# facebookresearch/foundpose

Hardware: AMD Instinct MI355X
Metric: detections/sec (ViT+kNN match) on 518^2 crops vs 10k-template bank (higher is better)
Workload: dtype bf16; 1 GPU; tie_order=torch

## Files before the change

### foundpose_amd/_lib.py

```python

import ctypes as C
import os

import torch

_HERE = os.path.dirname(os.path.abspath(__file__))
LIB_PATH = os.environ.get("FOUNDPOSE_AMD_LIB") or os.path.join(_HERE, "lib", "libfoundpose_amd.so")

FP_F32, FP_BF16, FP_FP8, FP_F16X3, FP_F16F8, FP_F16 = 0, 1, 2, 3, 4, 5
GEMM_SPLIT_F16F8 = 1 << 20
GEMM_F16 = 1 << 21
SPLIT_SCALE_ACT, SPLIT_SCALE_QKV, SPLIT_SCALE_HID = 16.0, 16.0, 4.0
ABI_VERSION = 20

vp, i32, i64, f32, f64, u64 = C.c_void_p, C.c_int, C.c_int64, C.c_float, C.c_double, C.c_uint64


class VitBlock(C.Structure):
    _fields_ = [(n, vp) for n in (
        "ln1_w", "ln1_b", "ln2_w", "ln2_b", "ls1", "ls2",
        "qkv_w", "proj_w", "fc1_w", "fc2_w",
        "qkv_b", "proj_b", "fc1_b", "fc2_b", "qkv_s", "proj_s", "fc1_s", "fc2_s")] + [("act_scale", f32 * 4), ("qkv_colsum", vp), ("fc1_colsum", vp)]


# ... 19 lines not shown
    "fp_normalize_rows": [vp, i64, i32, f32, vp, vp],
    "fp_knn_l2": [vp, vp, i32, vp, vp, i32, i32, i32, vp, vp, vp, vp],
    "fp_tfidf_build": [vp, vp, i32, vp, i32, vp, i32, i32, f32, i32, vp, vp, f32, vp],
    "fp_cosine_topk": [vp, vp, vp, i32, i32, vp, vp, i32, i32, i32, i32, vp, vp, vp, i32, vp],
    "fp_cosine_topk_prefiltered": [vp, vp, vp, i32, i32, vp, vp, vp, i32, i32, i32, i32, vp, vp, vp, i32, vp],
    "fp_cyclic_buddies": [vp, vp, vp, vp, i32, i32, vp, vp, vp, i32, vp, vp, vp, vp, i32, i32, i32, i32,
                          vp, vp, vp, vp, vp, vp, vp, vp, i32, vp],
    "fp_pack_records": [vp, vp, vp, vp, vp, vp, vp, vp, vp, i32, i32, i32, vp, vp],
    "fp_pnp_ransac": [vp, vp, vp, vp, i32, i32, i32, i32, f64, f64, i32, i32, u64, vp, vp, vp, vp, vp, vp, vp],
    "fp_sample_bilinear": [vp, i64, i64, i64, i64, i32, i32, i32, i32, i32, vp, vp, i32, vp, vp],
    "fp_pca_project": [vp, i32, i32, vp, i32, vp, vp, vp],
    "fp_vit_forward": [C.POINTER(VitModel), C.POINTER(VitWorkspace), vp, i32, i32, i32, i32, vp],
    "fp_vit_sample_features": [C.POINTER(VitModel), C.POINTER(VitWorkspace), i32, i32, i32, i32, i32, i32, vp, vp, i32, vp, vp],
    "fp_query_select": [vp, i32, i32, i32, vp, vp, vp, i32, vp, i32, i32, vp, vp, vp, vp, vp, vp, vp, vp, vp],
    "fp_vit_forward_prefix": [C.POINTER(VitModel), C.POINTER(VitWorkspace), vp, i32, i32, i32, i32, vp],
    "fp_vit_block_selected": [C.POINTER(VitModel), C.POINTER(VitWorkspace), i32, i32, i32, i32, vp, vp, i32, i32, vp],
    "fp_vit_sample_features_selected": [C.POINTER(VitModel), C.POINTER(VitWorkspace), i32, i32, i32, i32, i32, i32, vp, vp, i32, vp, vp, vp],
    "fp_vit_features": [C.POINTER(VitModel), C.POINTER(VitWorkspace), i32, i32, i32, vp, vp, vp],
    "fp_patchify": [vp, i32, i32, i32, i32, vp, i32, i32, vp],
    "fp_layernorm": [vp, i32, vp, vp, f32, vp, i32, i32, i32, i32, i32, i32, i32, vp],
    "fp_gemm_bf16": [vp, i32, vp, i32, i32, i32, i32, i32, vp, vp, vp, i32, i32, vp],
    "fp_gemm_bf16_ln": [vp, i32, vp, i32, i32, i32, i32, i32, vp, vp, i32, i32, vp, vp, vp, i32, vp, vp],
    "fp_gemm_resid_tile_rows": [i32, i32, i32],
    "fp_ln_finalize": [vp, i32, i32, i32, i32, f32, vp, vp],
    "fp_gemm_fp8": [vp, i32, vp, i32, i32, i32, i32, i32, vp, vp, vp, i32, i32, f32, vp],
    "fp_quantize_fp8": [vp, i32, i64, f32, vp, vp],
    "fp_gemm_split": [vp, i32, vp, i32, i32, i32, i32, i32, vp, vp, vp, i32, i32, f32, f32, vp],
    "fp_attention_split": [vp, i32, vp, i32, i32, i32, i32, i32, f32, f32, i32, vp],
    "fp_layernorm_scaled": [vp, i32, vp, vp, f32, vp, i32, i32, f32, i32, i32, vp],
    "fp_gemm_f32": [vp, i32, vp, i32, i32, i32, i32, vp, vp, vp, i32, i32, vp],
    "fp_attention": [vp, i32, vp, i32, i32, i32, i32, i32, i32, vp],
    "fp_convert_f32_to_bf16": [vp, vp, i64, vp],
    "fp_warp_crops": [vp, i32, i32, i32, i32, i32, vp, vp, i32, i32, i32, i32, vp, vp, vp],
    "fp_warp_depth": [vp, i32, i32, vp, vp, i32, i32, i32, i32, vp, vp],
    "fp_render_setup": [vp, vp, vp, i32, vp, i32, vp, i32, i32, i32, vp, vp, vp, vp, vp, vp, vp, vp, vp, vp, vp, vp],
    "fp_render_raster": [vp, vp, vp, i32, vp, i32, vp, i32, i32, i32, vp, vp, vp, vp, vp, vp, vp, vp, vp, vp, vp, vp],
    "fp_texture_mips": [vp, i32, i32, vp, vp],
    "fp_render_raster_textured": [vp, vp, vp, i32, vp, i32, vp, i32, i32, i32, vp, vp, vp, vp, vp, vp, vp, vp, vp, vp, vp, vp, vp,
                                  i32, i32, vp, vp],
    "fp_template_downsample": [vp, vp, vp, i32, i32, i32, i32, vp, vp, vp, vp, vp],
    "fp_pose_errors": [vp, i32, vp, vp, vp, vp, i32, vp, i32, vp, C.c_size_t, vp, vp, vp],
    "fp_vsd_counts": [vp, i32, vp, i32, vp, i32, i32, i32, vp, vp, i32, vp, i32, vp, C.c_size_t, vp, vp],
    "fp_featuremetric_refine": [vp, i64, i64, i64, i64, i32, i32, i32, i32, i32, vp, vp, vp, vp, vp, vp, vp, i64, vp, i32, i32, i32,
                                vp, C.c_size_t, vp, vp, vp, vp, vp, vp, vp, vp, vp],
    "fp_vis_pca_colorize": [vp, i32, i32, i32, i32, i32, i32, i32, i32, vp, vp, vp],
    "fp_vis_mask_tint": [vp, vp, i32, i32, i32, vp, vp],
# ... 130 lines not shown
```

### foundpose_amd/csrc/api.cpp

```cpp
#include <cstdarg>
#include <cstdio>
#include <cstring>
#include <cstdlib>
#include <vector>

#include "../../include/foundpose_amd.h"
#include "common.hpp"
#include "kernels.hpp"

static thread_local char g_err[512] = "";

void fp_set_error(const char* fmt, ...) {
  va_list ap;
  va_start(ap, fmt);
  vsnprintf(g_err, sizeof(g_err), fmt, ap);
  va_end(ap);
}

#define ST(s) reinterpret_cast<hipStream_t>(s)
#define TRY(expr)              \
  do {                         \
    int rc__ = (expr);         \
    if (rc__ != FP_OK) return rc__; \
  } while (0)
// ... 215 lines not shown
  return patchify_launch(images, B, H, W, patch, out, ld_out, out_dtype, ST(stream), (out_dtype == FP_DTYPE_F16X3 || out_dtype == FP_DTYPE_F16F8) ? FP_SPLIT_SCALE_ACT : 1.f);
}

int fp_layernorm(const float* x, int ld_x, const float* weight, const float* bias, float eps, void* out, int ld_out,
                 int out_dtype, int dim, int out_rows, int out_rows_per_img, int in_rows_per_img, int in_skip,
                 fp_stream_t stream) {
  FP_REQUIRE(x && weight && bias && out, "fp_layernorm: null pointer");
  LayerNormArgs a;
  memset(&a, 0, sizeof(a));
  a.x = x; a.ld_x = ld_x; a.weight = weight; a.bias = bias; a.eps = eps; a.out = out; a.ld_out = ld_out;
  a.out_dtype = out_dtype; a.out_scale = 0.f; a.dim = dim; a.out_rows = out_rows;
  a.out_rows_per_img = out_rows_per_img > 0 ? out_rows_per_img : (out_rows > 0 ? out_rows : 1);
  a.in_rows_per_img = in_rows_per_img > 0 ? in_rows_per_img : a.out_rows_per_img;
  a.in_skip = in_skip;
  return layernorm_launch(a, ST(stream));
}

int fp_gemm_bf16(const void* A, int lda, const void* W, int ldw, int M, int N, int K, int M_valid, const float* bias,
                 const float* gamma, void* out, int ldo, int epilogue, fp_stream_t stream) {
  FP_REQUIRE(A && W && out, "fp_gemm_bf16: null pointer");
  const int tile = (epilogue >> 8) & 0xfff;
  const bool f16 = (epilogue >> 21) & 1;
  epilogue &= 0xff;
  FP_REQUIRE(tile == 0 || tile == 64 || tile == 128 || tile == 256 || tile == 320, "fp_gemm_bf16: bad tile override %d", tile);

  FP_REQUIRE(epilogue == GEMM_EPI_BIAS_BF16 || epilogue == GEMM_EPI_GELU_BF16 || epilogue == GEMM_EPI_LS_RESID_F32 ||
                 epilogue == GEMM_EPI_BIAS_F32 || epilogue == GEMM_EPI_SWIGLU_BF16,
             "fp_gemm_bf16: epilogue %d is not available through this entry point", epilogue);
  FP_REQUIRE(epilogue != GEMM_EPI_LS_RESID_F32 || gamma, "fp_gemm_bf16: gamma required");
  GemmBf16Args a;
  memset(&a, 0, sizeof(a));
  a.A = reinterpret_cast<const __bf16*>(A); a.lda = lda; a.W = reinterpret_cast<const __bf16*>(W); a.ldw = ldw;
  a.M = M; a.N = N; a.K = K; a.M_valid = M_valid; a.bias = bias; a.gamma = gamma; a.out = out; a.ldo = ldo;
  a.tile_override = tile;
  return gemm_launch(f16 ? GemmFmt::F16 : GemmFmt::BF16, epilogue, a, ST(stream));
}

int fp_gemm_bf16_ln(const void* A, int lda, const void* W, int ldw, int M, int N, int K, int M_valid, const float* bias, void* out, int ldo,
                    int epilogue, const float* colsum, const float* ln_row, void* xb, int ld_xb, float* stats, fp_stream_t stream) {
  FP_REQUIRE(A && W && out && bias, "fp_gemm_bf16_ln: null pointer");
  const int tile = (epilogue >> 8) & 0xfff;
  const bool f16 = (epilogue >> 21) & 1;
  epilogue &= 0xff;
  FP_REQUIRE(tile == 0 || tile == 64 || tile == 128 || tile == 256 || tile == 320 || (tile == 352 && epilogue == GEMM_EPI_RESID_HILO), "fp_gemm_bf16_ln: bad tile override %d", tile);
  GemmBf16Args a;
  memset(&a, 0, sizeof(a));
  a.A = reinterpret_cast<const __bf16*>(A); a.lda = lda; a.W = reinterpret_cast<const __bf16*>(W); a.ldw = ldw;
  a.M = M; a.N = N; a.K = K; a.M_valid = M_valid; a.bias = bias; a.out = out; a.ldo = ldo; a.tile_override = tile;
  if (epilogue == GEMM_EPI_RESID_HILO) {
    FP_REQUIRE(xb && stats, "fp_gemm_bf16_ln: epilogue 8 needs xb, out (= the low halves) and stats");
    a.xb = reinterpret_cast<__bf16*>(xb); a.ld_xb = ld_xb; a.xl = reinterpret_cast<__bf16*>(out); a.stats_out = reinterpret_cast<float2*>(stats);
    a.out = nullptr;
  } else if (epilogue == GEMM_EPI_RESID_F32) {
    FP_REQUIRE((xb == nullptr) == (stats == nullptr), "fp_gemm_bf16_ln: xb and stats go together");
    FP_REQUIRE(!xb || (N % 128 == 0 && ld_xb >= N && ld_xb % 4 == 0), "fp_gemm_bf16_ln: N must be a multiple of 128 and ld_xb cover the row");
    a.xb = reinterpret_cast<__bf16*>(xb); a.ld_xb = ld_xb; a.stats_out = reinterpret_cast<float2*>(stats);
  } else {
    FP_REQUIRE(epilogue == GEMM_EPI_BIAS_BF16 || epilogue == GEMM_EPI_GELU_BF16 || epilogue == GEMM_EPI_SWIGLU_BF16,
               "fp_gemm_bf16_ln: epilogue %d has no folded-LayerNorm form", epilogue);
    FP_REQUIRE(colsum && ln_row, "fp_gemm_bf16_ln: colsum and ln_row are required");
    a.colsum = colsum; a.ln_stats = reinterpret_cast<const float2*>(ln_row); a.ln_eps = 1e-6f;
  }
  return gemm_launch(f16 ? GemmFmt::F16 : GemmFmt::BF16, epilogue, a, ST(stream));
}

int fp_gemm_resid_tile_rows(int M_valid, int N, int num_cus) { return gemm_resid_tile_rows(M_valid, N, num_cus); }

int fp_ln_finalize(const float* stats, int parts, int stats_stride, int rows, int dim, float eps, float* ln_row, fp_stream_t stream) {
  FP_REQUIRE(stats && ln_row && parts >= 1 && dim >= 1, "fp_ln_finalize: bad arguments");
  return ln_finalize_launch(reinterpret_cast<const float2*>(stats), parts, stats_stride, rows, dim, eps, reinterpret_cast<float2*>(ln_row), ST(stream));
}

#ifdef FP_GEMM_TIMELINE
int fp_gemm_bf16_timeline(const void* A, int lda, const void* W, int ldw, int M, int N, int K, int M_valid, const float* bias,
                          const float* gamma, void* out, int ldo, int epilogue, unsigned long long* dbg, int64_t dbg_len,
                          fp_stream_t stream) {
  FP_REQUIRE(A && W && out && dbg, "fp_gemm_bf16_timeline: null pointer");
  FP_REQUIRE(dbg_len >= 4ll * ((M + 127) / 128) * ((N + 127) / 128) * 2, "fp_gemm_bf16_timeline: stamp buffer too small");
  GemmBf16Args a;
  memset(&a, 0, sizeof(a));
  a.A = reinterpret_cast<const __bf16*>(A); a.lda = lda; a.W = reinterpret_cast<const __bf16*>(W); a.ldw = ldw;
  a.M = M; a.N = N; a.K = K; a.M_valid = M_valid; a.bias = bias; a.gamma = gamma; a.out = out; a.ldo = ldo;
  a.tile_override = (epilogue >> 8) & 0xfff;
  a.dbg = dbg;
  return gemm_launch(GemmFmt::BF16, epilogue & 0xff, a, ST(stream));
}
#endif

int fp_gemm_fp8(const void* A, int lda, const void* W, int ldw, int M, int N, int K, int M_valid, const float* bias,
// ... 635 lines not shown
```

### foundpose_amd/csrc/gemm_bf16.hip

```cpp
#include "gemm_kernel.hpp"

int gemm_resid_tile_rows(int m_valid, int n, int cus) { return resid_tile_rows(m_valid, n, cus); }

template int gemm_launch_fmt<GemmFmt::BF16>(int epi, const GemmBf16Args& a, hipStream_t st);
```

### foundpose_amd/csrc/gemm_kernel.hpp

```cpp
#pragma once
#include "common.hpp"
#include "kernels.hpp"
#include <type_traits>

namespace {

constexpr int BK = 64;

typedef __attribute__((address_space(3))) void lds_void;

FP_DEVICE int swz(int row) { return (row >> 1) & 7; }

FP_DEVICE unsigned stage_lane_offset(int ld, int lane, int parity) {
  const int row_l = lane >> 3;
  const int chunk = (lane & 7) ^ ((4 * parity + (row_l >> 1)) & 7);
  return (unsigned)(row_l * ld + chunk * 8) * 2u;
}
FP_DEVICE void stage_rows(__amdgpu_buffer_rsrc_t rsrc, unsigned voff, int ld, int row0, int k0, char* lds, int rblk) {
  const unsigned soff = (unsigned)((row0 + rblk * 8) * ld + k0) * 2u;
  __builtin_amdgcn_raw_ptr_buffer_load_lds(rsrc, (lds_void*)(lds + rblk * 1024), 16, voff, soff, 0, 0);
}

FP_DEVICE bf16x8 read_frag(const char* lds, int row, int chunk) {
  return *reinterpret_cast<const bf16x8*>(lds + row * 128 + ((chunk ^ swz(row)) << 4));
// ... 50 lines not shown
  q = __builtin_elementwise_fma(q, t, f32x2{0.15704123123125485f, 0.15704123123125485f});
  q = q * t;
  const f32x2 a = z * (z * f32x2{-1.44269504088896340736f, -1.44269504088896340736f});
  const f32x2 e = {__builtin_amdgcn_exp2f(a[0]), __builtin_amdgcn_exp2f(a[1])};
  const f32x2 erfz = __builtin_elementwise_fma(-q, e, f32x2{1.f, 1.f});
  return __builtin_elementwise_fma(hax, erfz, hx);
}

FP_DEVICE float row32_sum(float v) {
  v += __builtin_bit_cast(float, __builtin_amdgcn_update_dpp(0, __builtin_bit_cast(int, v), 0xB1, 0xF, 0xF, true));
  v += __builtin_bit_cast(float, __builtin_amdgcn_update_dpp(0, __builtin_bit_cast(int, v), 0x4E, 0xF, 0xF, true));
  v += __builtin_bit_cast(float, __builtin_amdgcn_update_dpp(0, __builtin_bit_cast(int, v), 0x124, 0xF, 0xF, true));
  v += __builtin_bit_cast(float, __builtin_amdgcn_update_dpp(0, __builtin_bit_cast(int, v), 0x128, 0xF, 0xF, true));
  v += __builtin_bit_cast(float, __builtin_amdgcn_update_dpp(0, __builtin_bit_cast(int, v), 0x142, 0xA, 0xF, true));
  return v;
}

FP_DEVICE float row16_sum(float v) {
  v += __builtin_bit_cast(float, __builtin_amdgcn_update_dpp(0, __builtin_bit_cast(int, v), 0xB1, 0xF, 0xF, true));
  v += __builtin_bit_cast(float, __builtin_amdgcn_update_dpp(0, __builtin_bit_cast(int, v), 0x4E, 0xF, 0xF, true));
  v += __builtin_bit_cast(float, __builtin_amdgcn_update_dpp(0, __builtin_bit_cast(int, v), 0x124, 0xF, 0xF, true));
  v += __builtin_bit_cast(float, __builtin_amdgcn_update_dpp(0, __builtin_bit_cast(int, v), 0x128, 0xF, 0xF, true));
  return v;
}

typedef __attribute__((ext_vector_type(8))) int i32x8;
typedef __attribute__((ext_vector_type(4))) int i32x4;

template <int EPI, int BM, int BN, int WM, int WN, GemmFmt FMT, bool F8OUT = false, int NSTAGE = 2>
__global__ __launch_bounds__(WM * WN * 64, 2) void gemm_bf16_kernel(GemmBf16Args a) {
  constexpr bool F8 = FMT == GemmFmt::FP8, SX = FMT == GemmFmt::F16F8, SP = FMT == GemmFmt::F16X3 || SX, H16 = FMT == GemmFmt::F16;
  constexpr bool SPOUT = SP && (EPI == GEMM_EPI_BIAS_BF16 || EPI == GEMM_EPI_GELU_BF16 || EPI == GEMM_EPI_SWIGLU_BF16);
  static_assert(NSTAGE == 2 || (NSTAGE == 4 && !F8 && !SP && WM * WN != 8), "the deep pipeline exists for the small bf16 / fp16 tiles");
  static_assert(!F8OUT || (F8 && (EPI == GEMM_EPI_GELU_BF16 || EPI == GEMM_EPI_SWIGLU_BF16)), "fp8 output: GELU / SwiGLU epilogues of the fp8 kernels");
  constexpr int NW = WM * WN, NT = NW * 64, MT = BM / 32, TM = (MT + WM - 1) / WM, WROWS = TM * 32, TN = BN / WN / 32;
  constexpr bool UNEVEN = MT % WM != 0;
  static_assert(BM % 32 == 0 && (!UNEVEN || (WM == 2 && FMT != GemmFmt::FP8 && FMT != GemmFmt::F16X3 && FMT != GemmFmt::F16F8)), "uneven wave rows: the bf16 / fp16 loop of the 2 x 4 wave grid");
  constexpr bool HILO = EPI == GEMM_EPI_RESID_HILO;
  constexpr bool RESID = EPI == GEMM_EPI_LS_RESID_F32 || EPI == GEMM_EPI_RESID_F32 || HILO;
  constexpr int A_BYTES = BM * BK * 2, B_BYTES = BN * BK * 2, STAGE = A_BYTES + B_BYTES;
  constexpr bool ASYM = NW == 8;
  constexpr int NISSUE = ASYM ? NW / 2 : NW;
  constexpr int A_INSTR = BM / 8 / NISSUE, B_INSTR = BN / 8 / NISSUE;
  constexpr int PIECES = A_INSTR + B_INSTR;
  static_assert(PIECES % 2 == 0 || !(F8 || SP), "staging split");
  extern __shared__ __attribute__((aligned(16))) char smem[];
// ... 43 lines not shown
    const unsigned voff_w[2] = {stage_lane_offset(a.ldw, lane, 0), stage_lane_offset(a.ldw, lane, 1)};
    const bool issuer = !ASYM || wm == 0;
    const int iw = ASYM ? wave % NISSUE : wave;
    const unsigned voff_a_w = voff_a[iw & 1];
    auto stage_piece = [&](int q, int t, char* buf) {
      if (!issuer) return;
      if (q < A_INSTR) {
        if constexpr (A_ILV) stage_rows(rsrc_a, voff_a_w, a.lda, 0, t * BK, buf, q * NISSUE + iw);
        else stage_rows(rsrc_a, voff_a[q & 1], a.lda, 0, t * BK, buf, iw * A_INSTR + q);
      }
      else stage_rows(rsrc_w, voff_w[(q - A_INSTR) & 1], a.ldw, 0, t * BK, buf + A_BYTES, iw * B_INSTR + (q - A_INSTR));
    };
#pragma unroll
    for (int q = 0; q < PIECES; ++q) stage_piece(q, kb, smem);
    if constexpr (NSTAGE > 2) {
#pragma unroll
      for (int d = 1; d < NSTAGE - 1; ++d)
        if (kb + d < ke) {
#pragma unroll
          for (int q = 0; q < PIECES; ++q) stage_piece(q, kb + d, smem + d * STAGE);
        }
    }

    float ln_rs[TM], ln_mrs[TM];
#pragma unroll
    for (int i = 0; i < TM; ++i) { ln_rs[i] = 1.f; ln_mrs[i] = 0.f; }
    if constexpr (!F8 && (EPI == GEMM_EPI_BIAS_BF16 || EPI == GEMM_EPI_GELU_BF16 || EPI == GEMM_EPI_SWIGLU_BF16)) {
      if (a.ln_stats) {
#pragma unroll
        for (int i = 0; i < TM; ++i) {
          if (!tile_on(i)) continue;
          const float2 st = a.ln_stats[m0 + wm * WROWS + i * 32 + l31];
          ln_rs[i] = st.x;
          ln_mrs[i] = st.y;
          if constexpr (H16) {
            ln_rs[i] *= a.acc_scale;
            ln_mrs[i] *= a.acc_scale;
          }
        }
      }
    }

    if constexpr (UNEVEN) {
      static_assert(NSTAGE == 2 && !F8 && !SP, "uneven wave rows: the two-stage bf16 / fp16 loop");
      auto k_loop = [&](auto tmw) {
        constexpr int TMW = decltype(tmw)::value;
        for (int t = kb; t < ke; ++t) {
          const int cur = (t - kb) & 1;
          asm volatile("s_waitcnt vmcnt(0)" ::: "memory");
          __syncthreads();
// ... 176 lines not shown
        }
      }
        }
      __syncthreads();
    }
#ifdef FP_GEMM_TIMELINE
    if (a.dbg) ts2 = __builtin_readcyclecounter();
#endif

    constexpr bool USE_SLAB = EPI == GEMM_EPI_BIAS_BF16 || EPI == GEMM_EPI_GELU_BF16 ||
                              EPI == GEMM_EPI_SWIGLU_BF16 || RESID;
    static_assert(!F8 || USE_SLAB, "the fp8 kernels exist for the slab epilogues only");
    if constexpr (USE_SLAB) {
    constexpr bool OUT_F32 = RESID || EPI == GEMM_EPI_TOKENS_F32 || EPI == GEMM_EPI_BIAS_F32;
    constexpr int ESZ = OUT_F32 ? 4 : (F8OUT ? 1 : (SPOUT ? 4 : 2));
    constexpr int OUT_COLS = EPI == GEMM_EPI_SWIGLU_BF16 ? BN / 2 : BN;
    constexpr int SLAB_ROWS = WM * 32, SLAB_STRIDE = OUT_COLS * ESZ + 16;
    constexpr int CHUNKS_PER_ROW = OUT_COLS * ESZ / 16, SLAB_CHUNKS = SLAB_ROWS * CHUNKS_PER_ROW, NT = NW * 64;
    static_assert(SLAB_ROWS * SLAB_STRIDE <= 2 * STAGE, "slab must fit the main-loop LDS");
    constexpr bool TWO_SLABS = 2 * SLAB_ROWS * SLAB_STRIDE <= 2 * STAGE;
    constexpr int SLAB_BYTES = SLAB_ROWS * SLAB_STRIDE;
    constexpr bool LN_FOLD_OK = !F8 && (EPI == GEMM_EPI_BIAS_BF16 || EPI == GEMM_EPI_GELU_BF16 || EPI == GEMM_EPI_SWIGLU_BF16);
    const bool fold = LN_FOLD_OK && a.ln_stats != nullptr;
    constexpr bool BIAS_LATE = TM * TN * 16 > 160;
    float4 bias[TN][4], gam[TN][4];
  #pragma unroll
    for (int tn = 0; tn < TN; ++tn)
  #pragma unroll
      for (int g = 0; g < 4; ++g) {
        const int n = n0 + wn * (BN / WN) + tn * 32 + 8 * g + 4 * kh;
        if constexpr (!BIAS_LATE) bias[tn][g] = *reinterpret_cast<const float4*>(a.bias + n);
        if constexpr (EPI == GEMM_EPI_LS_RESID_F32 || F8) gam[tn][g] = *reinterpret_cast<const float4*>(a.gamma + n);
        if constexpr (LN_FOLD_OK) {
          if (fold) gam[tn][g] = *reinterpret_cast<const float4*>(a.colsum + n);
        }
      }
    __syncthreads();
    float sat_amax = 0.f;
  #pragma unroll
    for (int tm = 0; tm < TM; ++tm) {
      const int m = m0 + wm * WROWS + tm * 32 + l31;
      float band_amax = 0.f;
      constexpr int PASSES = (SLAB_CHUNKS + NT - 1) / NT;
      static_assert(SLAB_CHUNKS % NT == 0, "slab chunks must divide evenly over the block");
      float4 ext[PASSES];
      int orow_i[PASSES];
      constexpr int CPR8 = HILO ? OUT_COLS / 8 : 1, PASS8 = HILO ? SLAB_ROWS * CPR8 / NT : 1;
      uint4 exh[PASS8], exl[PASS8];
      if constexpr (HILO) {
        static_assert(!HILO || (SLAB_ROWS * CPR8) % NT == 0, "slab chunks must divide evenly over the block");
  #pragma unroll
        for (int it = 0; it < PASS8; ++it) {
          const int id = tid + it * NT;
          const int r = id / CPR8, c = id - r * CPR8;
          const int gm_row = m0 + (r >> 5) * WROWS + tm * 32 + (r & 31);
          const bool okr = gm_row < a.M_valid && (!UNEVEN || (r >> 5) * TM + tm < MT);
          if (okr) {
            exh[it] = *reinterpret_cast<const uint4*>(a.xb + (size_t)gm_row * a.ld_xb + n0 + c * 8);
            exl[it] = *reinterpret_cast<const uint4*>(a.xl + (size_t)gm_row * a.ld_xb + n0 + c * 8);
          }
          orow_i[it] = okr ? gm_row : -1;
        }
      }
  #pragma unroll
      for (int it = 0; it < (HILO ? 0 : PASSES); ++it) {
        const int id = tid + it * NT;
        const int r = id / CHUNKS_PER_ROW, c = id - r * CHUNKS_PER_ROW;
        const int gm_row = m0 + (r >> 5) * WROWS + tm * 32 + (r & 31);
        const bool okr = gm_row < a.M_valid && (!UNEVEN || (r >> 5) * TM + tm < MT);
        int orow = gm_row;
        if constexpr (EPI == GEMM_EPI_TOKENS_F32) {
          const int b = gm_row / a.tok_np, pidx = gm_row - b * a.tok_np;
          orow = b * a.tok_n + a.tok_skip + pidx;
          if (okr) ext[it] = *reinterpret_cast<const float4*>(a.pos + (size_t)pidx * a.ldo + n0 + c * 4);
        }
        if constexpr (RESID) {
          if (okr) ext[it] = *reinterpret_cast<const float4*>(reinterpret_cast<const float*>(a.out) + (size_t)orow * a.ldo + n0 + c * 4);
        }
        orow_i[it] = okr ? orow : -1;
      }
      const float rs = ln_rs[tm], mrs = ln_mrs[tm];
      char* slab = smem + (TWO_SLABS ? (tm & 1) * SLAB_BYTES : 0);
      char* srow = slab + (wm * 32 + l31) * SLAB_STRIDE;
  #pragma unroll
      for (int tn = 0; tn < TN; ++tn)
  #pragma unroll
        for (int g = 0; g < 4; ++g) {
          const int col = wn * (BN / WN) + tn * 32 + 8 * g + 4 * kh;
          float4 bs;
          if constexpr (BIAS_LATE) bs = *reinterpret_cast<const float4*>(a.bias + n0 + col);
          else bs = bias[tn][g];
          float v0 = acc[tm][tn][4 * g + 0] + bs.x, v1 = acc[tm][tn][4 * g + 1] + bs.y;
          float v2 = acc[tm][tn][4 * g + 2] + bs.z, v3 = acc[tm][tn][4 * g + 3] + bs.w;
          if constexpr (SP || H16) {
            const float as = a.acc_scale;
            v0 = fmaf(acc[tm][tn][4 * g + 0], as, bs.x); v1 = fmaf(acc[tm][tn][4 * g + 1], as, bs.y);
            v2 = fmaf(acc[tm][tn][4 * g + 2], as, bs.z); v3 = fmaf(acc[tm][tn][4 * g + 3], as, bs.w);
          }
          if constexpr (LN_FOLD_OK) {
            if (fold) {
              const float4 cs = gam[tn][g];
              const f32x2 rs2 = {rs, rs}, nm2 = {-mrs, -mrs};
              const f32x2 t01 = __builtin_elementwise_fma(nm2, f32x2{cs.x, cs.y}, f32x2{bs.x, bs.y});
              const f32x2 t23 = __builtin_elementwise_fma(nm2, f32x2{cs.z, cs.w}, f32x2{bs.z, bs.w});
              const f32x2 r01 = __builtin_elementwise_fma(rs2, f32x2{acc[tm][tn][4 * g + 0], acc[tm][tn][4 * g + 1]}, t01);
              const f32x2 r23 = __builtin_elementwise_fma(rs2, f32x2{acc[tm][tn][4 * g + 2], acc[tm][tn][4 * g + 3]}, t23);
              v0 = r01[0]; v1 = r01[1]; v2 = r23[0]; v3 = r23[1];
            }
          }
          if constexpr (F8 && EPI != GEMM_EPI_LS_RESID_F32) {
            const float4 gm = gam[tn][g];
            v0 *= gm.x; v1 *= gm.y; v2 *= gm.z; v3 *= gm.w;
          }
          if constexpr (EPI == GEMM_EPI_GELU_BF16) {
            if constexpr (H16) {
              const f32x2 g01 = gelu_pk9(f32x2{v0, v1}), g23 = gelu_pk9(f32x2{v2, v3});
              v0 = g01[0]; v1 = g01[1]; v2 = g23[0]; v3 = g23[1];
            } else if constexpr (SP) {
              const f32x2 g01 = gelu_erf_pk(f32x2{v0, v1}), g23 = gelu_erf_pk(f32x2{v2, v3});
              v0 = g01[0]; v1 = g01[1]; v2 = g23[0]; v3 = g23[1];
            } else {
              const f32x2 g01 = gelu_pk(f32x2{v0, v1}), g23 = gelu_pk(f32x2{v2, v3});
              v0 = g01[0]; v1 = g01[1]; v2 = g23[0]; v3 = g23[1];
            }
// ... 205 lines not shown
  FP_CHECK_LAUNCH("gemm_bf16_kernel");
  return FP_OK;
}

static int xcd_rounds(int bm, int m_valid, int n_tiles, int cus) {
  const int m_tiles = (m_valid + bm - 1) / bm, xcds = 8, per_xcd = cus / xcds > 0 ? cus / xcds : 32;
  const GemmRaster ra = pick_raster(bm, n_tiles, (unsigned)(m_tiles * n_tiles));
  if (ra.r) return (((m_tiles + ra.r - 1) / ra.r) * (n_tiles / ra.gn) + xcds - 1) / xcds;
  const int chunk = (m_tiles * n_tiles + xcds - 1) / xcds;
  return (chunk + per_xcd - 1) / per_xcd;
}
static bool tall_tile_wins(const GemmBf16Args& a) {
  if (a.M % 320 != 0 || a.M % 256 != 0 || a.N % 256 != 0) return false;
  const int cus = fp_num_cus();
  return (float)(xcd_rounds(320, a.M_valid, a.N / 256, cus) * 320) * 0.97f < (float)(xcd_rounds(256, a.M_valid, a.N / 256, cus) * 256);
}

static int resid_tile_rows(int m_valid, int n, int cus) {
  if (m_valid <= 0 || n <= 0 || n % 256 != 0 || cus <= 0) return 256;
  const int r352 = xcd_rounds(352, m_valid, n / 256, cus), r256 = xcd_rounds(256, m_valid, n / 256, cus);
  return r352 < r256 && r352 * 352 < r256 * 256 ? 352 : 256;
}

template <int EPI, GemmFmt FMT>
int launch(const GemmBf16Args& a, hipStream_t st) {
  constexpr bool SP = FMT == GemmFmt::F16X3 || FMT == GemmFmt::F16F8;
  const int force = a.tile_override;
  const bool big_ok = a.M % 256 == 0 && a.N % 256 == 0;
  const int tiles_big = (a.M / 256) * (a.N / 256), cus = fp_num_cus();
  const bool use_big = big_ok && (force == 256 || (force == 0 && tiles_big >= cus && !(tiles_big > cus && tiles_big < cus + cus / 2)));
  if constexpr (!SP && (EPI == GEMM_EPI_BIAS_BF16 || EPI == GEMM_EPI_GELU_BF16 || EPI == GEMM_EPI_RESID_HILO)) {
    if ((force == 320 && a.M % 320 == 0 && a.N % 256 == 0) || (force == 0 && use_big && tall_tile_wins(a)))
      return launch_cfg<EPI, 320, 256, 2, 4, FMT>(a, st);
  }
  if constexpr (!SP && EPI == GEMM_EPI_RESID_HILO) {
    const bool ok352 = a.N % 256 == 0 && a.M_valid > 0 && a.M_valid <= a.M;
    if (ok352 && (force == 352 || (force == 0 && use_big && resid_tile_rows(a.M_valid, a.N, cus) == 352)))
      return launch_cfg<EPI, 352, 256, 2, 4, FMT>(a, st);
    FP_REQUIRE(force != 352, "gemm_bf16: the 352-row tile needs N %% 256 == 0 and 0 < M_valid <= M (N %d, M_valid %d, M %d)", a.N, a.M_valid, a.M);
  }
  if (use_big) return launch_cfg<EPI, 256, 256, 2, 4, FMT>(a, st);
  if constexpr (!SP && (EPI == GEMM_EPI_RESID_HILO || EPI == GEMM_EPI_RESID_F32 || EPI == GEMM_EPI_LS_RESID_F32)) {
    const int tiles_128 = (a.M_valid > 0 ? (a.M_valid + 127) / 128 : a.M / 128) * (a.N / 128);
    if ((force == 64 && a.M % 64 == 0) || (force == 0 && a.M % 64 == 0 && tiles_128 <= cus / 2))
      return launch_cfg<EPI, 64, 128, 2, 2, FMT, false, 4>(a, st);
  }
  return launch_cfg<EPI, 128, 128, 2, 2, FMT>(a, st);
}

template <int EPI, bool F8OUT = false>
int launch_fp8(const GemmBf16Args& a, hipStream_t st) {
  if constexpr (EPI != GEMM_EPI_LS_RESID_F32) {
    if (a.tile_override == 320 ? a.M % 320 == 0 : (a.tile_override == 0 && tall_tile_wins(a)))
      return launch_cfg<EPI, 320, 256, 2, 4, GemmFmt::FP8, F8OUT>(a, st);
  }
  return launch_cfg<EPI, 256, 256, 2, 4, GemmFmt::FP8, F8OUT>(a, st);
// ... 73 lines not shown
```

### foundpose_amd/csrc/kernels.hpp

```cpp
#pragma once
#include <hip/hip_runtime.h>
#include <stdint.h>

#include "../../include/foundpose_amd.h"

enum : int {
  F32_EPI_STORE = 0,
  F32_EPI_DIST_STORE = 1,
  F32_EPI_DIST_ARGMIN = 2,
  F32_EPI_SUB_VEC = 3,
  F32_EPI_BIAS = 4,
  F32_EPI_BIAS_GELU = 5,
  F32_EPI_LS_RESID = 6,
  F32_EPI_TOKENS = 7,
  F32_EPI_SWIGLU = 8,
  F32_EPI_DIST_TOPK = 9,
};

struct F32TileArgs {
  const float* A; int lda;
  const float* B; int ldb;
  int K, M, N;
  const int* a_seg_off; const int* pair_a_seg; int pair_a_div;
  const int* b_seg_off; const int* pair_b_seg;
// ... 111 lines not shown
  int tok_np, tok_n, tok_skip;
  int tile_override;
  int m_tiles;
  unsigned rast_r, rast_gn;
  float out_scale;
  float acc_scale;
  unsigned long long* dbg;
  __bf16* xb; int ld_xb;
  __bf16* xl;
  float2* stats_out;
  const float2* ln_stats; int ln_parts; float ln_eps;
  const float* colsum;
  int* sat;
};

enum class GemmFmt {
  BF16,
  F16,
  FP8,
  F16X3,
  F16F8,
};
template <GemmFmt FMT> int gemm_launch_fmt(int epi, const GemmBf16Args& a, hipStream_t st);
int gemm_resid_tile_rows(int m_valid, int n, int cus);
int gemm_launch(GemmFmt fmt, int epi, const GemmBf16Args& a, hipStream_t st);

enum : int { FP_DTYPE_F32 = 0, FP_DTYPE_BF16 = 1, FP_DTYPE_FP8 = 2, FP_DTYPE_F16X3 = 3, FP_DTYPE_F16F8 = 4,
             FP_DTYPE_F16 = 5 };

struct AttnArgs {
  const void* qkv; int ld_qkv;
  void* out; int ld_out;
  int batch, n_tok, dim, heads;
  float out_fp8_scale;
  const int* sel_rows; const int* sel_off; int max_sel;
  int variant;
  int tail_last;
  float in_scale, out_scale;
  int out_fmt;
  int* sat;
};
int attn_launch(const AttnArgs& a, int dtype, hipStream_t st);

struct LayerNormArgs {
  const float* x; int ld_x;
  const float* weight; const float* bias; float eps;
// ... 132 lines not shown
```

### foundpose_amd/ops.py

```python

from typing import Optional, Tuple

import torch

from . import _lib
from ._lib import call, knn_scratch_bytes, ptr, stream, require_cuda


def _f32c(t: torch.Tensor) -> torch.Tensor:
    if t.dtype != torch.float32:
        t = t.float()
    return t if t.is_contiguous() else t.contiguous()


def sqnorm_rows(x: torch.Tensor) -> torch.Tensor:
    require_cuda(x)
    x = _f32c(x)
    out = torch.empty(x.shape[0], dtype=torch.float32, device=x.device)
    call("fp_sqnorm_rows", ptr(x), x.shape[0], x.shape[1], ptr(out), stream())
    return out


def normalize_rows(x: torch.Tensor, eps: float = 1e-8) -> torch.Tensor:
    require_cuda(x)
# ... 74 lines not shown
    call("fp_pca_project", ptr(x), x.shape[0], x.shape[1], ptr(components), components.shape[0], ptr(mean_proj),
         ptr(out), stream())
    return out


def gemm_f32(a: torch.Tensor, w: torch.Tensor, bias=None, gamma=None, out=None, epilogue: int = 0) -> torch.Tensor:
    require_cuda(a, w)
    M, K = a.shape
    N = w.shape[0]
    if out is None:
        out = torch.empty(M, N, dtype=torch.float32, device=a.device)
    call("fp_gemm_f32", ptr(a), a.stride(0), ptr(w), w.stride(0), M, N, K, ptr(bias), ptr(gamma), ptr(out),
         out.stride(0), epilogue, stream())
    return out


def _h16_bit(a: torch.Tensor, w: torch.Tensor) -> int:
    if a.dtype != w.dtype or a.dtype not in (torch.bfloat16, torch.float16):
        raise ValueError("the 16-bit GEMMs take two bf16 or two fp16 operands")
    return _lib.GEMM_F16 if a.dtype == torch.float16 else 0


def gemm_bf16(a: torch.Tensor, w: torch.Tensor, bias: torch.Tensor, gamma=None, out=None, epilogue: int = 0,
              m_valid: Optional[int] = None) -> torch.Tensor:
    require_cuda(a, w, bias)
    M, K = a.shape
    N = w.shape[0]
    if out is None:
        dt = torch.float32 if (epilogue & 0xff) in (3, 5) else a.dtype
        out = torch.zeros(M, N // 2 if (epilogue & 0xff) == 6 else N, dtype=dt, device=a.device)
    call("fp_gemm_bf16", ptr(a), a.stride(0), ptr(w), w.stride(0), M, N, K, M if m_valid is None else m_valid,
         ptr(bias), ptr(gamma), ptr(out), out.stride(0), epilogue | _h16_bit(a, w), stream())
    return out


def gemm_bf16_resid_ln(a: torch.Tensor, w: torch.Tensor, bias: torch.Tensor, x: torch.Tensor, emit: bool = True, tile: int = 0, m_valid: Optional[int] = None):
    require_cuda(a, w, bias, x)
    M, K = a.shape
    N = w.shape[0]
    xb = torch.zeros(M, N, dtype=a.dtype, device=a.device) if emit else None
    stats = torch.zeros(N // 128, M, 2, dtype=torch.float32, device=a.device) if emit else None
    call("fp_gemm_bf16_ln", ptr(a), a.stride(0), ptr(w), w.stride(0), M, N, K, M if m_valid is None else m_valid, ptr(bias), ptr(x), x.stride(0),
         7 | (tile << 8) | _h16_bit(a, w), None, None, ptr(xb), N, ptr(stats), stream())
    return xb, stats


def gemm_bf16_resid_hilo(a: torch.Tensor, w: torch.Tensor, bias: torch.Tensor, xb: torch.Tensor, xl: torch.Tensor, tile: int = 0, m_valid: Optional[int] = None):
    require_cuda(a, w, bias, xb, xl)
    M, K = a.shape
    N = w.shape[0]
    if xb.dtype != a.dtype or xl.dtype != a.dtype or xb.stride(0) != xl.stride(0):
        raise ValueError("xb / xl are arrays of the operands' 16-bit type with one row stride")
    if xb.stride(0) % 8 or xb.data_ptr() % 16 or xl.data_ptr() % 16 or xb.stride(1) != 1 or xl.stride(1) != 1:
        raise ValueError("xb / xl: 16-byte aligned rows (row stride a multiple of 8 elements, unit column stride) -- the epilogue moves 8 bf16 per access")
    stats = torch.zeros(N // 128, M, 2, dtype=torch.float32, device=a.device)
# ... 221 lines not shown
```

### include/foundpose_amd.h

```cpp
#ifndef FOUNDPOSE_AMD_H
#define FOUNDPOSE_AMD_H

#include <stddef.h>
#include <stdint.h>

#ifdef __cplusplus
extern "C" {
#endif

typedef void* fp_stream_t;

enum { FP_F32 = 0, FP_BF16 = 1, FP_FP8 = 2, FP_F16X3 = 3, FP_F16F8 = 4, FP_F16 = 5 };

#define FP_SPLIT_SCALE_ACT 16.f
#define FP_SPLIT_SCALE_QKV 16.f
#define FP_SPLIT_SCALE_HID 4.f

#define FP_GEMM_SPLIT_F16F8 (1 << 20)

#define FP_GEMM_F16 (1 << 21)

#define FP_ABI_VERSION 20
int fp_abi_version(void);
const char* fp_last_error(void);
// ... 108 lines not shown
                           int img_h, const float* points, const int32_t* point_img, int num_points, float* out, fp_stream_t stream);

int fp_query_select(const uint8_t* masks, int B, int H, int W, const int32_t* pix_x, const int32_t* pix_y, const float* grid_points, int num_points,
                    const int64_t* point_cells, int num_cells, int n_tok, int32_t* scratch, int32_t* counts, float* out_points, int32_t* out_point_img,
                    int32_t* out_q_off, int32_t* sel_rows, int32_t* sel_off, int32_t* row_map, fp_stream_t stream);
int fp_vit_forward_prefix(const fp_vit_model* model, const fp_vit_workspace* ws, const float* images, int B, int H, int W, int layer,
                          fp_stream_t stream);
int fp_vit_block_selected(const fp_vit_model* model, const fp_vit_workspace* ws, int B, int H, int W, int layer, const int32_t* sel_rows,
                          const int32_t* sel_off, int num_sel, int max_sel_per_img, fp_stream_t stream);
int fp_vit_sample_features_selected(const fp_vit_model* model, const fp_vit_workspace* ws, int B, int grid_h, int grid_w, int apply_norm,
                                    int img_w, int img_h, const float* points, const int32_t* point_img, int num_points,
                                    const int32_t* row_map, float* out, fp_stream_t stream);

int fp_patchify(const float* images, int B, int H, int W, int patch, void* out, int ld_out, int out_dtype,
                fp_stream_t stream);
int fp_layernorm(const float* x, int ld_x, const float* weight, const float* bias, float eps, void* out, int ld_out,
                 int out_dtype, int dim, int out_rows, int out_rows_per_img, int in_rows_per_img, int in_skip,
                 fp_stream_t stream);
int fp_gemm_bf16(const void* A, int lda, const void* W, int ldw, int M, int N, int K, int M_valid, const float* bias,
                 const float* gamma, void* out, int ldo, int epilogue, fp_stream_t stream);
int fp_gemm_bf16_ln(const void* A, int lda, const void* W, int ldw, int M, int N, int K, int M_valid, const float* bias, void* out, int ldo,
                    int epilogue, const float* colsum, const float* ln_row, void* xb, int ld_xb, float* stats, fp_stream_t stream);
int fp_gemm_resid_tile_rows(int M_valid, int N, int num_cus);
int fp_ln_finalize(const float* stats, int parts, int stats_stride, int rows, int dim, float eps, float* ln_row, fp_stream_t stream);

int fp_gemm_fp8(const void* A, int lda, const void* W, int ldw, int M, int N, int K, int M_valid, const float* bias,
                const float* col_scale, void* out, int ldo, int epilogue, float out_scale, fp_stream_t stream);
int fp_gemm_split(const void* A, int lda, const void* W, int ldw, int M, int N, int K, int M_valid, const float* bias, const float* gamma,
                  void* out, int ldo, int epilogue, float acc_scale, float out_scale, fp_stream_t stream);
int fp_attention_split(const void* qkv, int ld_qkv, void* out, int ld_out, int B, int n_tok, int dim, int heads, float in_scale, float out_scale,
                       int out_dtype, fp_stream_t stream);
int fp_layernorm_scaled(const float* x, int ld_x, const float* weight, const float* bias, float eps, void* out, int ld_out, int out_dtype, float out_scale,
                        int dim, int out_rows, fp_stream_t stream);
int fp_quantize_fp8(const void* in, int in_dtype, int64_t n, float scale, void* out, fp_stream_t stream);
int fp_gemm_f32(const float* A, int lda, const float* W, int ldw, int M, int N, int K, const float* bias,
                const float* gamma, float* out, int ldo, int epilogue, fp_stream_t stream);
#define FP_ATTN_VARIANT(v) ((v) << 8)
int fp_attention(const void* qkv, int ld_qkv, void* out, int ld_out, int B, int n_tok,
                 int dim, int heads, int dtype, fp_stream_t stream);
int fp_convert_f32_to_bf16(const float* in, void* out, int64_t n, fp_stream_t stream);

enum { FP_WARP_LINEAR = 0, FP_WARP_NEAREST = 1 };
int fp_warp_crops(const void* src, int n_src, int src_h, int src_w, int channels, int mode, const int32_t* src_index,
                  const double* params, int batch, int out_h, int out_w, int depth_check, void* out, float* map_out,
                  fp_stream_t stream);

// ... 79 lines not shown
```

Baseline: 1161 detections/s.

## Enable 320/352-row GEMM tiles for bias and GELU epilogues with late LN stats

```diff
diff --git a/foundpose_amd/_lib.py b/foundpose_amd/_lib.py
--- a/foundpose_amd/_lib.py
+++ b/foundpose_amd/_lib.py
@@ -65,6 +65,7 @@
     "fp_gemm_bf16": [vp, i32, vp, i32, i32, i32, i32, i32, vp, vp, vp, i32, i32, vp],
     "fp_gemm_bf16_ln": [vp, i32, vp, i32, i32, i32, i32, i32, vp, vp, i32, i32, vp, vp, vp, i32, vp, vp],
     "fp_gemm_resid_tile_rows": [i32, i32, i32],
+    "fp_gemm_wide_tile_rows": [i32, i32, i32, i32, i32],
     "fp_ln_finalize": [vp, i32, i32, i32, i32, f32, vp, vp],
     "fp_gemm_fp8": [vp, i32, vp, i32, i32, i32, i32, i32, vp, vp, vp, i32, i32, f32, vp],
     "fp_quantize_fp8": [vp, i32, i64, f32, vp, vp],
diff --git a/foundpose_amd/csrc/api.cpp b/foundpose_amd/csrc/api.cpp
--- a/foundpose_amd/csrc/api.cpp
+++ b/foundpose_amd/csrc/api.cpp
@@ -261,7 +261,8 @@
   const int tile = (epilogue >> 8) & 0xfff;
   const bool f16 = (epilogue >> 21) & 1;
   epilogue &= 0xff;
-  FP_REQUIRE(tile == 0 || tile == 64 || tile == 128 || tile == 256 || tile == 320, "fp_gemm_bf16: bad tile override %d", tile);
+  FP_REQUIRE(tile == 0 || tile == 64 || tile == 128 || tile == 256 || tile == 320 || (tile == 352 && (epilogue == GEMM_EPI_BIAS_BF16 || epilogue == GEMM_EPI_GELU_BF16)),
+             "fp_gemm_bf16: bad tile override %d (352 rows: epilogues 0 and 1)", tile);
 
   FP_REQUIRE(epilogue == GEMM_EPI_BIAS_BF16 || epilogue == GEMM_EPI_GELU_BF16 || epilogue == GEMM_EPI_LS_RESID_F32 ||
                  epilogue == GEMM_EPI_BIAS_F32 || epilogue == GEMM_EPI_SWIGLU_BF16,
@@ -281,7 +282,8 @@
   const int tile = (epilogue >> 8) & 0xfff;
   const bool f16 = (epilogue >> 21) & 1;
   epilogue &= 0xff;
-  FP_REQUIRE(tile == 0 || tile == 64 || tile == 128 || tile == 256 || tile == 320 || (tile == 352 && epilogue == GEMM_EPI_RESID_HILO), "fp_gemm_bf16_ln: bad tile override %d", tile);
+  FP_REQUIRE(tile == 0 || tile == 64 || tile == 128 || tile == 256 || tile == 320 || (tile == 352 && (epilogue == GEMM_EPI_RESID_HILO || epilogue == GEMM_EPI_BIAS_BF16 || epilogue == GEMM_EPI_GELU_BF16)),
+             "fp_gemm_bf16_ln: bad tile override %d (352 rows: epilogues 0, 1 and 8)", tile);
   GemmBf16Args a;
   memset(&a, 0, sizeof(a));
   a.A = reinterpret_cast<const __bf16*>(A); a.lda = lda; a.W = reinterpret_cast<const __bf16*>(W); a.ldw = ldw;
@@ -304,6 +306,7 @@
 }
 
 int fp_gemm_resid_tile_rows(int M_valid, int N, int num_cus) { return gemm_resid_tile_rows(M_valid, N, num_cus); }
+int fp_gemm_wide_tile_rows(int epilogue, int M, int M_valid, int N, int num_cus) { return gemm_wide_tile_rows(epilogue, M, M_valid, N, num_cus); }
 
 int fp_ln_finalize(const float* stats, int parts, int stats_stride, int rows, int dim, float eps, float* ln_row, fp_stream_t stream) {
   FP_REQUIRE(stats && ln_row && parts >= 1 && dim >= 1, "fp_ln_finalize: bad arguments");
diff --git a/foundpose_amd/csrc/gemm_bf16.hip b/foundpose_amd/csrc/gemm_bf16.hip
--- a/foundpose_amd/csrc/gemm_bf16.hip
+++ b/foundpose_amd/csrc/gemm_bf16.hip
@@ -1,5 +1,6 @@
 #include "gemm_kernel.hpp"
 
 int gemm_resid_tile_rows(int m_valid, int n, int cus) { return resid_tile_rows(m_valid, n, cus); }
+int gemm_wide_tile_rows(int epi, int m, int m_valid, int n, int cus) { return wide_tile_rows(epi, m, m_valid, n, cus); }
 
 template int gemm_launch_fmt<GemmFmt::BF16>(int epi, const GemmBf16Args& a, hipStream_t st);
diff --git a/foundpose_amd/csrc/gemm_kernel.hpp b/foundpose_amd/csrc/gemm_kernel.hpp
--- a/foundpose_amd/csrc/gemm_kernel.hpp
+++ b/foundpose_amd/csrc/gemm_kernel.hpp
@@ -96,6 +96,15 @@
   v += __builtin_bit_cast(float, __builtin_amdgcn_update_dpp(0, __builtin_bit_cast(int, v), 0x124, 0xF, 0xF, true));
   v += __builtin_bit_cast(float, __builtin_amdgcn_update_dpp(0, __builtin_bit_cast(int, v), 0x128, 0xF, 0xF, true));
   return v;
+}
+
+FP_DEVICE float2 ln_late_fetch(const float2* stats, bool on, int row, float scale) {
+  float2 st = make_float2(1.f, 0.f);
+  if (on) {
+    st = stats[row];
+    st.x *= scale; st.y *= scale;
+  }
+  return st;
 }
 
 typedef __attribute__((ext_vector_type(8))) int i32x8;
@@ -185,10 +194,11 @@
         }
     }
 
+    constexpr bool EPI_LATE = TM * TN * 16 > 160;
     float ln_rs[TM], ln_mrs[TM];
 #pragma unroll
     for (int i = 0; i < TM; ++i) { ln_rs[i] = 1.f; ln_mrs[i] = 0.f; }
-    if constexpr (!F8 && (EPI == GEMM_EPI_BIAS_BF16 || EPI == GEMM_EPI_GELU_BF16 || EPI == GEMM_EPI_SWIGLU_BF16)) {
+    if constexpr (!EPI_LATE && !F8 && (EPI == GEMM_EPI_BIAS_BF16 || EPI == GEMM_EPI_GELU_BF16 || EPI == GEMM_EPI_SWIGLU_BF16)) {
       if (a.ln_stats) {
 #pragma unroll
         for (int i = 0; i < TM; ++i) {
@@ -411,7 +421,7 @@
     constexpr int SLAB_BYTES = SLAB_ROWS * SLAB_STRIDE;
     constexpr bool LN_FOLD_OK = !F8 && (EPI == GEMM_EPI_BIAS_BF16 || EPI == GEMM_EPI_GELU_BF16 || EPI == GEMM_EPI_SWIGLU_BF16);
     const bool fold = LN_FOLD_OK && a.ln_stats != nullptr;
-    constexpr bool BIAS_LATE = TM * TN * 16 > 160;
+    constexpr bool BIAS_LATE = EPI_LATE;
     float4 bias[TN][4], gam[TN][4];
   #pragma unroll
     for (int tn = 0; tn < TN; ++tn)
@@ -420,10 +430,15 @@
         const int n = n0 + wn * (BN / WN) + tn * 32 + 8 * g + 4 * kh;
         if constexpr (!BIAS_LATE) bias[tn][g] = *reinterpret_cast<const float4*>(a.bias + n);
         if constexpr (EPI == GEMM_EPI_LS_RESID_F32 || F8) gam[tn][g] = *reinterpret_cast<const float4*>(a.gamma + n);
-        if constexpr (LN_FOLD_OK) {
+        if constexpr (LN_FOLD_OK && !BIAS_LATE) {
           if (fold) gam[tn][g] = *reinterpret_cast<const float4*>(a.colsum + n);
         }
       }
+    float2 ln_nxt;
+    if constexpr (BIAS_LATE && LN_FOLD_OK) {
+      const int row = m0 + wm * WROWS + l31;
+      ln_nxt = ln_late_fetch(a.ln_stats, fold && row < a.M_valid, row, H16 ? a.acc_scale : 1.f);
+    }
     __syncthreads();
     float sat_amax = 0.f;
   #pragma unroll
@@ -468,7 +483,11 @@
         }
         orow_i[it] = okr ? orow : -1;
       }
-      const float rs = ln_rs[tm], mrs = ln_mrs[tm];
+      float rs = ln_rs[tm], mrs = ln_mrs[tm];
+      if constexpr (BIAS_LATE && LN_FOLD_OK) {
+        rs = ln_nxt.x; mrs = ln_nxt.y;
+        if (tm + 1 < TM) ln_nxt = ln_late_fetch(a.ln_stats, fold && tile_on(tm + 1) && m + 32 < a.M_valid, m + 32, H16 ? a.acc_scale : 1.f);
+      }
       char* slab = smem + (TWO_SLABS ? (tm & 1) * SLAB_BYTES : 0);
       char* srow = slab + (wm * 32 + l31) * SLAB_STRIDE;
   #pragma unroll
@@ -488,7 +507,9 @@
           }
           if constexpr (LN_FOLD_OK) {
             if (fold) {
-              const float4 cs = gam[tn][g];
+              float4 cs;
+              if constexpr (BIAS_LATE) cs = *reinterpret_cast<const float4*>(a.colsum + n0 + col);
+              else cs = gam[tn][g];
               const f32x2 rs2 = {rs, rs}, nm2 = {-mrs, -mrs};
               const f32x2 t01 = __builtin_elementwise_fma(nm2, f32x2{cs.x, cs.y}, f32x2{bs.x, bs.y});
               const f32x2 t23 = __builtin_elementwise_fma(nm2, f32x2{cs.z, cs.w}, f32x2{bs.z, bs.w});
@@ -740,6 +761,22 @@
   return r352 < r256 && r352 * 352 < r256 * 256 ? 352 : 256;
 }
 
+constexpr float WIDE_F320 = 0.97f, WIDE_F352 = 1.02f, WIDE_MARGIN = 0.01f;
+static int wide_tile_rows(int epi, int m, int m_valid, int n, int cus) {
+  if ((epi != GEMM_EPI_BIAS_BF16 && epi != GEMM_EPI_GELU_BF16) || m <= 0 || m_valid <= 0 || m_valid > m || n <= 0 || n % 256 != 0 || cus <= 0) return 256;
+  const int nt = n / 256;
+  const float c256 = (float)(xcd_rounds(256, m_valid, nt, cus) * 256);
+  int best = 256;
+  float cost = c256;
+  if (m % 320 == 0 && m % 256 == 0) {
+    const float c320 = (float)(xcd_rounds(320, m_valid, nt, cus) * 320) * WIDE_F320;
+    if (c320 < c256) { best = 320; cost = c320; }
+  }
+  const float c352 = (float)(xcd_rounds(352, m_valid, nt, cus) * 352) * WIDE_F352;
+  if (c352 < cost * (1.f - WIDE_MARGIN)) best = 352;
+  return best;
+}
+
 template <int EPI, GemmFmt FMT>
 int launch(const GemmBf16Args& a, hipStream_t st) {
   constexpr bool SP = FMT == GemmFmt::F16X3 || FMT == GemmFmt::F16F8;
@@ -747,9 +784,17 @@
   const bool big_ok = a.M % 256 == 0 && a.N % 256 == 0;
   const int tiles_big = (a.M / 256) * (a.N / 256), cus = fp_num_cus();
   const bool use_big = big_ok && (force == 256 || (force == 0 && tiles_big >= cus && !(tiles_big > cus && tiles_big < cus + cus / 2)));
-  if constexpr (!SP && (EPI == GEMM_EPI_BIAS_BF16 || EPI == GEMM_EPI_GELU_BF16 || EPI == GEMM_EPI_RESID_HILO)) {
+  if constexpr (!SP && (EPI == GEMM_EPI_BIAS_BF16 || EPI == GEMM_EPI_GELU_BF16)) {
+    const int rows = force == 0 && use_big ? wide_tile_rows(EPI, a.M, a.M_valid, a.N, cus) : 0;
+    const bool ok352 = a.N % 256 == 0 && a.M_valid > 0 && a.M_valid <= a.M;
+    FP_REQUIRE(force != 352 || ok352, "gemm_bf16: the 352-row tile needs N %% 256 == 0 and 0 < M_valid <= M (N %d, M_valid %d, M %d)", a.N, a.M_valid, a.M);
+    if (force == 352 || rows == 352) return launch_cfg<EPI, 352, 256, 2, 4, FMT>(a, st);
+    if ((force == 320 && a.M % 320 == 0 && a.N % 256 == 0) || rows == 320) return launch_cfg<EPI, 320, 256, 2, 4, FMT>(a, st);
+  } else if constexpr (!SP && EPI == GEMM_EPI_RESID_HILO) {
     if ((force == 320 && a.M % 320 == 0 && a.N % 256 == 0) || (force == 0 && use_big && tall_tile_wins(a)))
       return launch_cfg<EPI, 320, 256, 2, 4, FMT>(a, st);
+  } else {
+    FP_REQUIRE(force != 352, "gemm_bf16: the 352-row tile exists for the bf16 / fp16 BIAS, GELU and (hi, lo) residual epilogues (epilogue %d)", EPI);
   }
   if constexpr (!SP && EPI == GEMM_EPI_RESID_HILO) {
     const bool ok352 = a.N % 256 == 0 && a.M_valid > 0 && a.M_valid <= a.M;
diff --git a/foundpose_amd/csrc/kernels.hpp b/foundpose_amd/csrc/kernels.hpp
--- a/foundpose_amd/csrc/kernels.hpp
+++ b/foundpose_amd/csrc/kernels.hpp
@@ -157,6 +157,7 @@
   F16F8,
 };
 template <GemmFmt FMT> int gemm_launch_fmt(int epi, const GemmBf16Args& a, hipStream_t st);
+int gemm_wide_tile_rows(int epi, int m, int m_valid, int n, int cus);
 int gemm_resid_tile_rows(int m_valid, int n, int cus);
 int gemm_launch(GemmFmt fmt, int epi, const GemmBf16Args& a, hipStream_t st);
 
diff --git a/foundpose_amd/ops.py b/foundpose_amd/ops.py
--- a/foundpose_amd/ops.py
+++ b/foundpose_amd/ops.py
@@ -120,7 +120,7 @@
 
 
 def gemm_bf16(a: torch.Tensor, w: torch.Tensor, bias: torch.Tensor, gamma=None, out=None, epilogue: int = 0,
-              m_valid: Optional[int] = None) -> torch.Tensor:
+              m_valid: Optional[int] = None, tile: int = 0) -> torch.Tensor:
     require_cuda(a, w, bias)
     M, K = a.shape
     N = w.shape[0]
@@ -128,7 +128,7 @@
         dt = torch.float32 if (epilogue & 0xff) in (3, 5) else a.dtype
         out = torch.zeros(M, N // 2 if (epilogue & 0xff) == 6 else N, dtype=dt, device=a.device)
     call("fp_gemm_bf16", ptr(a), a.stride(0), ptr(w), w.stride(0), M, N, K, M if m_valid is None else m_valid,
-         ptr(bias), ptr(gamma), ptr(out), out.stride(0), epilogue | _h16_bit(a, w), stream())
+         ptr(bias), ptr(gamma), ptr(out), out.stride(0), epilogue | (tile << 8) | _h16_bit(a, w), stream())
     return out
 
 
diff --git a/include/foundpose_amd.h b/include/foundpose_amd.h
--- a/include/foundpose_amd.h
+++ b/include/foundpose_amd.h
@@ -154,6 +154,7 @@
 int fp_gemm_bf16_ln(const void* A, int lda, const void* W, int ldw, int M, int N, int K, int M_valid, const float* bias, void* out, int ldo,
                     int epilogue, const float* colsum, const float* ln_row, void* xb, int ld_xb, float* stats, fp_stream_t stream);
 int fp_gemm_resid_tile_rows(int M_valid, int N, int num_cus);
+int fp_gemm_wide_tile_rows(int epilogue, int M, int M_valid, int N, int num_cus);
 int fp_ln_finalize(const float* stats, int parts, int stats_stride, int rows, int dim, float eps, float* ln_row, fp_stream_t stream);
 
 int fp_gemm_fp8(const void* A, int lda, const void* W, int ldw, int M, int N, int K, int M_valid, const float* bias,
```

Measured after the change: 1160 detections/s. No clear change (-0.1%).
